# Haochen-Wang409/U2PL

Hardware: AMD Instinct MI355X
Metric: train images/sec at 769x769 (R101-DeepLabv3+) (higher is better)
Workload: dtype f32

## Files before the change

### u2pl_amd/csrc/nn.hip

```cpp
#include "common.h"
#include "u2pl_hip.h"

__device__ __forceinline__ float4 f4add(float4 a, float4 b) { return make_float4(a.x + b.x, a.y + b.y, a.z + b.z, a.w + b.w); }
__device__ __forceinline__ float4 f4mul(float4 a, float4 b) { return make_float4(a.x * b.x, a.y * b.y, a.z * b.z, a.w * b.w); }
__device__ __forceinline__ float4 f4sub(float4 a, float4 b) { return make_float4(a.x - b.x, a.y - b.y, a.z - b.z, a.w - b.w); }
__device__ __forceinline__ float4 f4zero() { return make_float4(0.f, 0.f, 0.f, 0.f); }

struct StatOp {
    const float* x; long ld; const float* pivot;
    __device__ __forceinline__ void get(long row, int c4, float4& v0, float4& v1) const {
        float4 v = *(const float4*)(x + row * ld + c4 * 4);
        if (pivot) v = f4sub(v, *(const float4*)(pivot + c4 * 4));
        v0 = v; v1 = f4mul(v, v);
    }
};
struct SumOp {
    const float* x; long ld;
    __device__ __forceinline__ void get(long row, int c4, float4& v0, float4& v1) const {
        v0 = *(const float4*)(x + row * ld + c4 * 4); v1 = f4zero();
    }
};
__device__ __forceinline__ float4 relu_mask_from_x(float4 g, float4 xv, const float* mean, const float* invstd, const float* gamma,
                                                   const float* beta, int c) {
    const float4 mu = *(const float4*)(mean + c), is = *(const float4*)(invstd + c), ga = *(const float4*)(gamma + c), be = *(const float4*)(beta + c);
    g.x = ((xv.x - mu.x) * is.x * ga.x + be.x) > 0.f ? g.x : 0.f;
    g.y = ((xv.y - mu.y) * is.y * ga.y + be.y) > 0.f ? g.y : 0.f;
    g.z = ((xv.z - mu.z) * is.z * ga.z + be.z) > 0.f ? g.z : 0.f;
    g.w = ((xv.w - mu.w) * is.w * ga.w + be.w) > 0.f ? g.w : 0.f;
    return g;
}
struct BnBwdOp {
    const float* dy; long lddy; const float* x; long ldx; const float* y; long ldy;
    const float* mean; const float* invstd; const float* drop; long rows_per_image; int C;
    const float* gamma; const float* relu_beta;
    __device__ __forceinline__ void get(long row, int c4, float4& v0, float4& v1) const {
        float4 g = *(const float4*)(dy + row * lddy + c4 * 4);
        float4 xv = *(const float4*)(x + row * ldx + c4 * 4);
        if (y) {
            float4 yy = *(const float4*)(y + row * ldy + c4 * 4);
            g.x = yy.x > 0.f ? g.x : 0.f; g.y = yy.y > 0.f ? g.y : 0.f;
            g.z = yy.z > 0.f ? g.z : 0.f; g.w = yy.w > 0.f ? g.w : 0.f;
        } else if (relu_beta) {
            g = relu_mask_from_x(g, xv, mean, invstd, gamma, relu_beta, c4 * 4);
        }
        if (drop) g = f4mul(g, *(const float4*)(drop + (row / rows_per_image) * C + c4 * 4));
        float4 xh = f4mul(f4sub(xv, *(const float4*)(mean + c4 * 4)), *(const float4*)(invstd + c4 * 4));
        v0 = g; v1 = f4mul(g, xh);
    }
};

template <class Op>
__global__ U2PL_HBM_KERNEL void k_colreduce_partial(Op op, long Mseg, int C, float* __restrict__ partial) {
    __shared__ float4 sh0[256], sh1[256];
    const int C4 = C >> 2;
    const int slab0 = blockIdx.z * 64;
    const int wcols = min(64, C4 - slab0);
    const int tc = wcols, tr = 256 / tc;
    const int tid = threadIdx.x, cl = tid % tc, rg = tid / tc;
    const int nblk = gridDim.x, seg = blockIdx.y;
    const long per = (Mseg + nblk - 1) / nblk;
    const long rb = seg * Mseg + blockIdx.x * per, re = min(seg * Mseg + Mseg, rb + per);
    float* out = partial + ((long)seg * nblk + blockIdx.x) * 2 * C;
    const int c4 = slab0 + cl;
    float4 a0 = f4zero(), a1 = f4zero();
    if (rg < tr) {
        float4 b0 = f4zero(), b1 = f4zero(), c0 = f4zero(), c1 = f4zero(), d0 = f4zero(), d1 = f4zero();
        long r = rb + rg;
        for (; r + 3 * (long)tr < re; r += 4 * (long)tr) {
            float4 v0, v1, w0, w1, x0, x1, y0, y1;
            op.get(r, c4, v0, v1);
            op.get(r + tr, c4, w0, w1);
            op.get(r + 2 * (long)tr, c4, x0, x1);
            op.get(r + 3 * (long)tr, c4, y0, y1);
            a0 = f4add(a0, v0); a1 = f4add(a1, v1);
            b0 = f4add(b0, w0); b1 = f4add(b1, w1);
            c0 = f4add(c0, x0); c1 = f4add(c1, x1);
            d0 = f4add(d0, y0); d1 = f4add(d1, y1);
        }
        for (; r < re; r += tr) {
            float4 v0, v1;
            op.get(r, c4, v0, v1);
            a0 = f4add(a0, v0); a1 = f4add(a1, v1);
        }
        a0 = f4add(f4add(a0, b0), f4add(c0, d0));
        a1 = f4add(f4add(a1, b1), f4add(c1, d1));
    }
    sh0[tid] = a0; sh1[tid] = a1;
    __syncthreads();
    if (rg == 0) {
        for (int k = 1; k < tr; ++k) { a0 = f4add(a0, sh0[k * tc + cl]); a1 = f4add(a1, sh1[k * tc + cl]); }
        *(float4*)(out + c4 * 4) = a0;
        *(float4*)(out + C + c4 * 4) = a1;
    }
}
__global__ __launch_bounds__(1024) void k_colreduce_final(const float* __restrict__ partial, int nblk, int C,
                                                          double* __restrict__ out) {
    __shared__ double sh[16][64];
    const int seg = blockIdx.y;
    const int cl = threadIdx.x & 63, rg = threadIdx.x >> 6;
    const int i = blockIdx.x * 64 + cl;
    double acc = 0.0;
    if (i < 2 * C) {
        const float* p = partial + (long)seg * nblk * 2 * C + i;
        int b = rg;
        for (; b + 7 * 16 < nblk; b += 8 * 16) {
            float v[8];
#pragma unroll
            for (int u = 0; u < 8; ++u) v[u] = p[(long)(b + u * 16) * 2 * C];
#pragma unroll
            for (int u = 0; u < 8; ++u) acc += (double)v[u];
        }
        for (; b < nblk; b += 16) acc += (double)p[(long)b * 2 * C];
    }
    sh[rg][cl] = acc;
    __syncthreads();
    if (rg == 0 && i < 2 * C) {
        double t = 0.0;
#pragma unroll
        for (int k = 0; k < 16; ++k) t += sh[k][cl];
        out[(long)seg * 2 * C + i] = t;
    }
}
static int colreduce_blocks(long Mseg) {
    long b = (Mseg + 63) / 64;
    return (int)(b < 1 ? 1 : (b > 512 ? 512 : b));
}
U2PL_API size_t u2pl_colreduce_workspace_bytes(long Mseg, int nseg, int C) {
    return (size_t)nseg * colreduce_blocks(Mseg) * 2 * C * sizeof(float);
}
template <class Op>
static int run_colreduce(Op op, long Mseg, int nseg, int C, void* ws, double* out, hipStream_t stream) {
    if (C % 4 || Mseg <= 0) return U2PL_EINVAL;
    const int nblk = colreduce_blocks(Mseg);
    U2PL_LAUNCH((k_colreduce_partial<Op>), dim3(nblk, nseg, cdiv(C / 4, 64)), dim3(256), 0, stream, op, Mseg, C, (float*)ws);
    U2PL_LAUNCH_CHECK();
    U2PL_LAUNCH(k_colreduce_final, dim3(cdiv(2 * C, 64), nseg), dim3(1024), 0, stream, (const float*)ws, nblk, C, out);
    U2PL_LAUNCH_CHECK();
    return 0;
}

U2PL_API int u2pl_colreduce_finish_f32(const float* partial, int nblk, int C, double* sums, hipStream_t stream) {
    U2PL_LAUNCH(k_colreduce_final, dim3(cdiv(2 * C, 64), 1), dim3(1024), 0, stream, partial, nblk, C, sums);
    U2PL_LAUNCH_CHECK();
    return 0;
}

__global__ void k_bn_stats_small(const float* __restrict__ x, long ld, int M, int C, const float* __restrict__ pivot,
                                 double* __restrict__ sums) {
    const int c = blockIdx.x * blockDim.x + threadIdx.x;
    if (c >= C) return;
    double s = 0.0;
    for (int m = 0; m < M; ++m) s += (double)x[m * ld + c];
    const double mean = s / M;
    double q = 0.0;
    for (int m = 0; m < M; ++m) { const double d = (double)x[m * ld + c] - mean; q += d * d; }
    const double dm = mean - (pivot ? (double)pivot[c] : 0.0);
    sums[c] = M * dm;
    sums[C + c] = q + M * dm * dm;
}
U2PL_API int u2pl_bn_stats_f32(const float* x, long ld, long M, int C, const float* pivot, void* workspace,
                               double* sums, hipStream_t stream) {
    if (M <= 64) {
        U2PL_LAUNCH(k_bn_stats_small, dim3(cdiv(C, 64)), dim3(64), 0, stream, x, ld, (int)M, C, pivot, sums);
        U2PL_LAUNCH_CHECK();
        return 0;
    }
    StatOp op = {x, ld, pivot};
    return run_colreduce(op, M, 1, C, workspace, sums, stream);
}
U2PL_API int u2pl_colsum_f32(const float* x, long ld, long Mseg, int nseg, int C, void* workspace, double* sums,
                             hipStream_t stream) {
    SumOp op = {x, ld};
    return run_colreduce(op, Mseg, nseg, C, workspace, sums, stream);
}
U2PL_API int u2pl_bn_bwd_sums_f32(const float* dy, long lddy, const float* x, long ldx, const float* y, long ldy,
                                  const float* mean, const float* invstd, const float* drop, long rows_per_image,
                                  long M, int C, void* workspace, double* sums, hipStream_t stream) {
    BnBwdOp op = {dy, lddy, x, ldx, y, ldy, mean, invstd, drop, rows_per_image, C, nullptr, nullptr};
    return run_colreduce(op, M, 1, C, workspace, sums, stream);
}
U2PL_API int u2pl_bn_bwd_sums_mx_f32(const float* dy, long lddy, const float* x, long ldx, const float* mean, const float* invstd,
                                     const float* gamma, const float* beta, const float* drop, long rows_per_image, long M, int C,
                                     void* workspace, double* sums, hipStream_t stream) {
    if (!gamma || !beta) return U2PL_EINVAL;
    BnBwdOp op = {dy, lddy, x, ldx, nullptr, 0, mean, invstd, drop, rows_per_image, C, gamma, beta};
    return run_colreduce(op, M, 1, C, workspace, sums, stream);
}

__global__ void k_bn_finalize(const double* __restrict__ sums, double count, const float* __restrict__ pivot, int C,
                              float eps, float momentum, float* __restrict__ mean, float* __restrict__ invstd,
                              float* __restrict__ running_mean, float* __restrict__ running_var) {
    for (int c = blockIdx.x * blockDim.x + threadIdx.x; c < C; c += gridDim.x * blockDim.x) {
        const double m1 = sums[c] / count, m2 = sums[C + c] / count;
        const double p = pivot ? (double)pivot[c] : 0.0;
        double var = m2 - m1 * m1;
        if (var < 0.0) var = 0.0;
        const double mu = p + m1;
        mean[c] = (float)mu;
        invstd[c] = (float)(1.0 / sqrt(var + (double)eps));
        if (running_mean) {
            const double unb = count > 1.0 ? var * count / (count - 1.0) : var;
            running_mean[c] = (float)((1.0 - momentum) * running_mean[c] + momentum * mu);
            running_var[c] = (float)((1.0 - momentum) * running_var[c] + momentum * unb);
        }
    }
}
U2PL_API int u2pl_bn_finalize_f32(const double* sums, double count, const float* pivot, int C, float eps,
                                  float momentum, float* mean, float* invstd, float* running_mean,
                                  float* running_var, hipStream_t stream) {
    U2PL_LAUNCH(k_bn_finalize, dim3(cdiv(C, 256)), dim3(256), 0, stream, sums, count, pivot, C, eps, momentum,
                       mean, invstd, running_mean, running_var);
    U2PL_LAUNCH_CHECK();
    return 0;
}
__global__ __launch_bounds__(1024) void k_bn_finish_finalize(const float* __restrict__ partial, int nblk, int C, double count,
                                                             const float* __restrict__ pivot, float eps, float momentum,
                                                             float* __restrict__ mean, float* __restrict__ invstd,
                                                             float* __restrict__ running_mean, float* __restrict__ running_var,
                                                             double* __restrict__ sums_out) {
    __shared__ double sh[16][64];
    __shared__ double tot[64];
    const int cl = threadIdx.x & 63, rg = threadIdx.x >> 6;
    const int c = blockIdx.x * 32 + (cl & 31);
    const int i = (cl >> 5) * C + c;
    double acc = 0.0;
    if (c < C) {
        const float* p = partial + i;
        int b = rg;
        for (; b + 7 * 16 < nblk; b += 8 * 16) {
            float v[8];
#pragma unroll
            for (int u = 0; u < 8; ++u) v[u] = p[(long)(b + u * 16) * 2 * C];
#pragma unroll
            for (int u = 0; u < 8; ++u) acc += (double)v[u];
        }
        for (; b < nblk; b += 16) acc += (double)p[(long)b * 2 * C];
    }
    sh[rg][cl] = acc;
    __syncthreads();
    if (rg == 0) {
        double t = 0.0;
#pragma unroll
        for (int k = 0; k < 16; ++k) t += sh[k][cl];
        tot[cl] = t;
        if (sums_out && c < C) sums_out[i] = t;
    }
    __syncthreads();
    if (threadIdx.x < 32 && c < C) {
        const double m1 = tot[cl] / count, m2 = tot[32 + cl] / count;
        const double pv = pivot ? (double)pivot[c] : 0.0;
        double var = m2 - m1 * m1;
        if (var < 0.0) var = 0.0;
        const double mu = pv + m1;
        mean[c] = (float)mu;
        invstd[c] = (float)(1.0 / sqrt(var + (double)eps));
        if (running_mean) {
            const double unb = count > 1.0 ? var * count / (count - 1.0) : var;
            running_mean[c] = (float)((1.0 - momentum) * running_mean[c] + momentum * mu);
            running_var[c] = (float)((1.0 - momentum) * running_var[c] + momentum * unb);
        }
    }
}
U2PL_API int u2pl_bn_finish_finalize_f32(const float* partial, int nblk, int C, double count, const float* pivot, float eps,
                                         float momentum, float* mean, float* invstd, float* running_mean, float* running_var,
                                         double* sums_out, hipStream_t stream) {
    if (!partial || nblk <= 0 || C <= 0 || !mean || !invstd) return U2PL_EINVAL;
    U2PL_LAUNCH(k_bn_finish_finalize, dim3(cdiv(C, 32)), dim3(1024), 0, stream, partial, nblk, C, count, pivot, eps, momentum, mean,
                invstd, running_mean, running_var, sums_out);
    U2PL_LAUNCH_CHECK();
    return 0;
}
__global__ void k_bn_eval_prep(const float* __restrict__ rv, int C, float eps, float* __restrict__ invstd) {
    for (int c = blockIdx.x * blockDim.x + threadIdx.x; c < C; c += gridDim.x * blockDim.x)
        invstd[c] = (float)(1.0 / sqrt((double)rv[c] + (double)eps));
}
U2PL_API int u2pl_bn_eval_invstd_f32(const float* running_var, int C, float eps, float* invstd, hipStream_t stream) {
    U2PL_LAUNCH(k_bn_eval_prep, dim3(cdiv(C, 256)), dim3(256), 0, stream, running_var, C, eps, invstd);
    U2PL_LAUNCH_CHECK();
    return 0;
}

struct EvalPrepJob { const float* rv; float* out; long long begin; int C; float eps; };
__global__ void k_bn_eval_prep_multi(const EvalPrepJob* __restrict__ jobs, int njobs, long total) {
    for (long e = blockIdx.x * (long)blockDim.x + threadIdx.x; e < total; e += (long)gridDim.x * blockDim.x) {
        int lo = 0, hi = njobs - 1;
        while (lo < hi) {
            const int mid = (lo + hi + 1) >> 1;
            if (jobs[mid].begin <= e) lo = mid; else hi = mid - 1;
        }
        const EvalPrepJob j = jobs[lo];
        const int c = (int)(e - j.begin);
        if (c < j.C) j.out[c] = (float)(1.0 / sqrt((double)j.rv[c] + (double)j.eps));
    }
}
U2PL_API size_t u2pl_bn_eval_invstd_job_bytes(void) { return sizeof(EvalPrepJob); }
U2PL_API int u2pl_bn_eval_invstd_multi_f32(const void* jobs_dev, int njobs, long total, hipStream_t stream) {
    if (njobs <= 0 || total <= 0) return 0;
    if (!jobs_dev) return U2PL_EINVAL;
    U2PL_LAUNCH(k_bn_eval_prep_multi, dim3(grid_for(total, 256)), dim3(256), 0, stream, (const EvalPrepJob*)jobs_dev, njobs, total);
    U2PL_LAUNCH_CHECK();
    return 0;
}

__global__ U2PL_HBM_KERNEL void k_bn_apply(const float* __restrict__ x, long ldx, const float* __restrict__ mean,
                           const float* __restrict__ invstd, const float* __restrict__ gamma,
                           const float* __restrict__ beta, const float* __restrict__ res, long ldr, int relu,
                           const float* __restrict__ drop, long rows_per_image, float* __restrict__ y, long ldy,
                           long M, int C, unsigned* __restrict__ y_amax) {
    const int C4 = C >> 2;
    const long total = M * C4;
    unsigned am = 0u;
    for (long i = blockIdx.x * (long)blockDim.x + threadIdx.x; i < total; i += (long)gridDim.x * blockDim.x) {
        const long r = i / C4;
        const int c = (int)(i % C4) * 4;
        float4 v = *(const float4*)(x + r * ldx + c);
        const float4 mu = *(const float4*)(mean + c), is = *(const float4*)(invstd + c);
        const float4 ga = *(const float4*)(gamma + c), be = *(const float4*)(beta + c);
        v.x = (v.x - mu.x) * is.x * ga.x + be.x; v.y = (v.y - mu.y) * is.y * ga.y + be.y;
        v.z = (v.z - mu.z) * is.z * ga.z + be.z; v.w = (v.w - mu.w) * is.w * ga.w + be.w;
        if (res) v = f4add(v, *(const float4*)(res + r * ldr + c));
        if (relu) { v.x = fmaxf(v.x, 0.f); v.y = fmaxf(v.y, 0.f); v.z = fmaxf(v.z, 0.f); v.w = fmaxf(v.w, 0.f); }
        if (drop) v = f4mul(v, *(const float4*)(drop + (r / rows_per_image) * C + c));
        *(float4*)(y + r * ldy + c) = v;
        am = amax_bits4(am, v);
    }
    if (y_amax) amax_wave_publish(am, y_amax);
}
U2PL_API int u2pl_bn_apply_f32(const float* x, long ldx, const float* mean, const float* invstd, const float* gamma,
                               const float* beta, const float* res, long ldr, int relu, const float* drop,
                               long rows_per_image, float* y, long ldy, long M, int C, hipStream_t stream) {
    if (C % 4) return U2PL_EINVAL;
    U2PL_LAUNCH(k_bn_apply, dim3(grid_for(M * (C / 4), 256)), dim3(256), 0, stream, x, ldx, mean, invstd, gamma,
                       beta, res, ldr, relu, drop, rows_per_image, y, ldy, M, C, (unsigned*)nullptr);
    U2PL_LAUNCH_CHECK();
    return 0;
}
U2PL_API int u2pl_bn_apply_amax_f32(const float* x, long ldx, const float* mean, const float* invstd, const float* gamma,
                                    const float* beta, const float* res, long ldr, int relu, const float* drop,
                                    long rows_per_image, float* y, long ldy, long M, int C, float* y_amax, hipStream_t stream) {
    if (C % 4) return U2PL_EINVAL;
    U2PL_LAUNCH(k_bn_apply, dim3(grid_for(M * (C / 4), 256)), dim3(256), 0, stream, x, ldx, mean, invstd, gamma,
                       beta, res, ldr, relu, drop, rows_per_image, y, ldy, M, C, (unsigned*)y_amax);
    U2PL_LAUNCH_CHECK();
    return 0;
}

__global__ U2PL_HBM_KERNEL void k_bn_bwd_apply(const float* __restrict__ dy, long lddy, const float* __restrict__ x, long ldx,
                               const float* __restrict__ y, long ldy, const float* __restrict__ mean,
                               const float* __restrict__ invstd, const float* __restrict__ gamma,
                               const float* __restrict__ drop, long rows_per_image,
                               const double* __restrict__ sums, double count, float* __restrict__ dx, long lddx,
                               float* __restrict__ dres, long lddr, long M, int C, const double* __restrict__ psums,
                               float* __restrict__ gsink, float* __restrict__ bsink, int accumulate,
                               unsigned* __restrict__ dx_amax, unsigned* __restrict__ dres_amax, const float* __restrict__ relu_beta) {
    unsigned am_x = 0u, am_r = 0u;
    if (psums) {
        for (long i = blockIdx.x * (long)blockDim.x + threadIdx.x; i < C; i += (long)gridDim.x * blockDim.x) {
            gsink[i] = (accumulate ? gsink[i] : 0.f) + (float)(psums[C + i] * (double)1.0f);
            bsink[i] = (accumulate ? bsink[i] : 0.f) + (float)(psums[i] * (double)1.0f);
        }
    }
    const int C4 = C >> 2;
    const long total = M * C4;
    for (long i = blockIdx.x * (long)blockDim.x + threadIdx.x; i < total; i += (long)gridDim.x * blockDim.x) {
        const long r = i / C4;
        const int c = (int)(i % C4) * 4;
        float4 g = *(const float4*)(dy + r * lddy + c);
        if (y) {
            const float4 yy = *(const float4*)(y + r * ldy + c);
            g.x = yy.x > 0.f ? g.x : 0.f; g.y = yy.y > 0.f ? g.y : 0.f;
            g.z = yy.z > 0.f ? g.z : 0.f; g.w = yy.w > 0.f ? g.w : 0.f;
        } else if (relu_beta) {
            g = relu_mask_from_x(g, *(const float4*)(x + r * ldx + c), mean, invstd, gamma, relu_beta, c);
        }
        if (drop) g = f4mul(g, *(const float4*)(drop + (r / rows_per_image) * C + c));
        if (dres) *(float4*)(dres + r * lddr + c) = g;
        am_r = amax_bits4(am_r, g);
        const float4 is = *(const float4*)(invstd + c), ga = *(const float4*)(gamma + c);
        float4 o;
        if (sums) {
            const float4 xv = *(const float4*)(x + r * ldx + c), mu = *(const float4*)(mean + c);
            const float m0x = (float)(sums[c] / count), m0y = (float)(sums[c + 1] / count);
            const float m0z = (float)(sums[c + 2] / count), m0w = (float)(sums[c + 3] / count);
            const float m1x = (float)(sums[C + c] / count), m1y = (float)(sums[C + c + 1] / count);
            const float m1z = (float)(sums[C + c + 2] / count), m1w = (float)(sums[C + c + 3] / count);
            o.x = ga.x * is.x * (g.x - m0x - (xv.x - mu.x) * is.x * m1x);
            o.y = ga.y * is.y * (g.y - m0y - (xv.y - mu.y) * is.y * m1y);
            o.z = ga.z * is.z * (g.z - m0z - (xv.z - mu.z) * is.z * m1z);
            o.w = ga.w * is.w * (g.w - m0w - (xv.w - mu.w) * is.w * m1w);
        } else {
            o = f4mul(f4mul(ga, is), g);
        }
        *(float4*)(dx + r * lddx + c) = o;
        am_x = amax_bits4(am_x, o);
    }
    if (dx_amax) amax_wave_publish(am_x, dx_amax);
    if (dres_amax) amax_wave_publish(am_r, dres_amax);
}
U2PL_API int u2pl_bn_bwd_apply_f32(const float* dy, long lddy, const float* x, long ldx, const float* y, long ldy,
                                   const float* mean, const float* invstd, const float* gamma, const float* drop,
                                   long rows_per_image, const double* sums, double count, float* dx, long lddx,
                                   float* dres, long lddr, long M, int C, hipStream_t stream) {
    if (C % 4) return U2PL_EINVAL;
    U2PL_LAUNCH(k_bn_bwd_apply, dim3(grid_for(M * (C / 4), 256)), dim3(256), 0, stream, dy, lddy, x, ldx, y, ldy,
                       mean, invstd, gamma, drop, rows_per_image, sums, count, dx, lddx, dres, lddr, M, C, (const double*)nullptr,
                       (float*)nullptr, (float*)nullptr, 0, (unsigned*)nullptr, (unsigned*)nullptr, (const float*)nullptr);
    U2PL_LAUNCH_CHECK();
    return 0;
}
U2PL_API int u2pl_bn_bwd_apply_pg_f32(const float* dy, long lddy, const float* x, long ldx, const float* y, long ldy,
                                      const float* mean, const float* invstd, const float* gamma, const float* drop,
                                      long rows_per_image, const double* sums, double count, float* dx, long lddx,
                                      float* dres, long lddr, long M, int C, const double* psums, float* gsink, float* bsink,
                                      int accumulate, hipStream_t stream) {
    if (C % 4 || !psums || !gsink || !bsink) return U2PL_EINVAL;
    U2PL_LAUNCH(k_bn_bwd_apply, dim3(grid_for(M * (C / 4), 256)), dim3(256), 0, stream, dy, lddy, x, ldx, y, ldy,
                       mean, invstd, gamma, drop, rows_per_image, sums, count, dx, lddx, dres, lddr, M, C, psums, gsink, bsink,
                       accumulate, (unsigned*)nullptr, (unsigned*)nullptr, (const float*)nullptr);
    U2PL_LAUNCH_CHECK();
    return 0;
}
U2PL_API int u2pl_bn_bwd_apply_amax_f32(const float* dy, long lddy, const float* x, long ldx, const float* y, long ldy,
                                        const float* mean, const float* invstd, const float* gamma, const float* drop,
                                        long rows_per_image, const double* sums, double count, float* dx, long lddx,
                                        float* dres, long lddr, long M, int C, const double* psums, float* gsink, float* bsink,
                                        int accumulate, float* dx_amax, float* dres_amax, const float* relu_beta, hipStream_t stream) {
    if (C % 4 || (psums && (!gsink || !bsink)) || (relu_beta && y)) return U2PL_EINVAL;
    U2PL_LAUNCH(k_bn_bwd_apply, dim3(grid_for(M * (C / 4), 256)), dim3(256), 0, stream, dy, lddy, x, ldx, y, ldy,
                       mean, invstd, gamma, drop, rows_per_image, sums, count, dx, lddx, dres, lddr, M, C, psums, gsink, bsink,
                       accumulate, (unsigned*)dx_amax, (unsigned*)dres_amax, relu_beta);
    U2PL_LAUNCH_CHECK();
    return 0;
}
__global__ void k_sums_to_f32(const double* __restrict__ s, int n, float scale, int accumulate, float* __restrict__ out) {
    for (int i = blockIdx.x * blockDim.x + threadIdx.x; i < n; i += gridDim.x * blockDim.x)
        out[i] = (accumulate ? out[i] : 0.f) + (float)(s[i] * (double)scale);
}
U2PL_API int u2pl_sums_to_f32(const double* sums, int n, float scale, int accumulate, float* out, hipStream_t stream) {
    U2PL_LAUNCH(k_sums_to_f32, dim3(cdiv(n, 256)), dim3(256), 0, stream, sums, n, scale, accumulate, out);
    U2PL_LAUNCH_CHECK();
    return 0;
}

__global__ void k_maxpool_fwd(const float* __restrict__ x, long ldx, int N, int H, int W, int C, int Ho, int Wo,
                              float* __restrict__ y, long ldy, unsigned char* __restrict__ tap) {
    const int C4 = C >> 2;
    const long total = (long)N * Ho * Wo * C4;
    for (long i = blockIdx.x * (long)blockDim.x + threadIdx.x; i < total; i += (long)gridDim.x * blockDim.x) {
        const int c = (int)(i % C4) * 4;
        long p = i / C4;
        const int wo = (int)(p % Wo);
        long t = p / Wo;
        const int ho = (int)(t % Ho), n = (int)(t / Ho);
        float4 best = make_float4(-INFINITY, -INFINITY, -INFINITY, -INFINITY);
        uchar4 bt = make_uchar4(0, 0, 0, 0);
        bool first = true;
        for (int r = 0; r < 3; ++r) {
            const int ih = ho * 2 - 1 + r;
            if (ih < 0 || ih >= H) continue;
            for (int s = 0; s < 3; ++s) {
                const int iw = wo * 2 - 1 + s;
                if (iw < 0 || iw >= W) continue;
                const float4 v = *(const float4*)(x + ((long)(n * H + ih) * W + iw) * ldx + c);
                const unsigned char k = (unsigned char)(r * 3 + s);
                if (first || v.x > best.x || v.x != v.x) { best.x = v.x; bt.x = k; }
                if (first || v.y > best.y || v.y != v.y) { best.y = v.y; bt.y = k; }
                if (first || v.z > best.z || v.z != v.z) { best.z = v.z; bt.z = k; }
                if (first || v.w > best.w || v.w != v.w) { best.w = v.w; bt.w = k; }
                first = false;
            }
        }
        *(float4*)(y + p * ldy + c) = best;
        *(uchar4*)(tap + p * C + c) = bt;
    }
}
U2PL_API int u2pl_maxpool3s2_fwd_f32(const float* x, long ldx, int N, int H, int W, int C, int Ho, int Wo, float* y,
                                     long ldy, unsigned char* tap, hipStream_t stream) {
    if (C % 4) return U2PL_EINVAL;
    U2PL_LAUNCH(k_maxpool_fwd, dim3(grid_for((long)N * Ho * Wo * (C / 4), 256)), dim3(256), 0, stream, x, ldx, N, H,
                       W, C, Ho, Wo, y, ldy, tap);
    U2PL_LAUNCH_CHECK();
    return 0;
}
__global__ void k_maxpool_bwd(const float* __restrict__ dy, long lddy, const unsigned char* __restrict__ tap, int N,
                              int H, int W, int C, int Ho, int Wo, float* __restrict__ dx, long lddx) {
    const int C4 = C >> 2;
    const long total = (long)N * H * W * C4;
    for (long i = blockIdx.x * (long)blockDim.x + threadIdx.x; i < total; i += (long)gridDim.x * blockDim.x) {
        const int c = (int)(i % C4) * 4;
        long p = i / C4;
        const int iw = (int)(p % W);
        long t = p / W;
        const int ih = (int)(t % H), n = (int)(t / H);
        float4 acc = f4zero();
        for (int ho = ih / 2; ho <= (ih + 1) / 2; ++ho) {
            if (ho >= Ho) continue;
            const int r = ih - (ho * 2 - 1);
            if (r < 0 || r > 2) continue;
            for (int wo = iw / 2; wo <= (iw + 1) / 2; ++wo) {
                if (wo >= Wo) continue;
                const int s = iw - (wo * 2 - 1);
                if (s < 0 || s > 2) continue;
                const long q = ((long)n * Ho + ho) * Wo + wo;
                const uchar4 k = *(const uchar4*)(tap + q * C + c);
                const float4 g = *(const float4*)(dy + q * lddy + c);
                const unsigned char me = (unsigned char)(r * 3 + s);
                if (k.x == me) acc.x += g.x;
                if (k.y == me) acc.y += g.y;
                if (k.z == me) acc.z += g.z;
                if (k.w == me) acc.w += g.w;
            }
        }
        *(float4*)(dx + p * lddx + c) = acc;
    }
}
U2PL_API int u2pl_maxpool3s2_bwd_f32(const float* dy, long lddy, const unsigned char* tap, int N, int H, int W, int C,
                                     int Ho, int Wo, float* dx, long lddx, hipStream_t stream) {
    U2PL_LAUNCH(k_maxpool_bwd, dim3(grid_for((long)N * H * W * (C / 4), 256)), dim3(256), 0, stream, dy, lddy, tap, N,
                       H, W, C, Ho, Wo, dx, lddx);
    U2PL_LAUNCH_CHECK();
    return 0;
}

__global__ void k_copy_rows(const float* __restrict__ src, long lds, float* __restrict__ dst, long ldd, long M, int C,
                            int accumulate) {
    const int C4 = C >> 2;
    const long total = M * C4;
    for (long i = blockIdx.x * (long)blockDim.x + threadIdx.x; i < total; i += (long)gridDim.x * blockDim.x) {
        const long r = i / C4;
        const int c = (int)(i % C4) * 4;
        float4 v = *(const float4*)(src + r * lds + c);
        if (accumulate) v = f4add(v, *(const float4*)(dst + r * ldd + c));
        *(float4*)(dst + r * ldd + c) = v;
    }
}
U2PL_API int u2pl_copy_rows_f32(const float* src, long lds, float* dst, long ldd, long M, int C, int accumulate,
                                hipStream_t stream) {
    if (C % 4) return U2PL_EINVAL;
    if (M <= 0) return 0;
    U2PL_LAUNCH(k_copy_rows, dim3(grid_for(M * (C / 4), 256)), dim3(256), 0, stream, src, lds, dst, ldd, M, C, accumulate);
    U2PL_LAUNCH_CHECK();
    return 0;
}
__global__ void k_copy_cols(const float* __restrict__ src, long lds, float* __restrict__ dst, long ldd, long M, int C) {
    const long total = M * C;
    for (long i = blockIdx.x * (long)blockDim.x + threadIdx.x; i < total; i += (long)gridDim.x * blockDim.x) {
        const long r = i / C;
        const int c = (int)(i % C);
        dst[r * ldd + c] = src[r * lds + c];
    }
}
U2PL_API int u2pl_copy_cols_f32(const float* src, long lds, float* dst, long ldd, long M, int C, hipStream_t stream) {
    if (M <= 0) return 0;
    U2PL_LAUNCH(k_copy_cols, dim3(grid_for(M * C, 256)), dim3(256), 0, stream, src, lds, dst, ldd, M, C);
    U2PL_LAUNCH_CHECK();
    return 0;
}
__global__ void k_broadcast_rows(const float* __restrict__ v, long ldv, float scale, float* __restrict__ dst, long ldd,
                                 long rows_per_image, long M, int C) {
    const int C4 = C >> 2;
    const long total = M * C4;
    for (long i = blockIdx.x * (long)blockDim.x + threadIdx.x; i < total; i += (long)gridDim.x * blockDim.x) {
        const long r = i / C4;
        const int c = (int)(i % C4) * 4;
        float4 a = *(const float4*)(v + (r / rows_per_image) * ldv + c);
        a.x *= scale; a.y *= scale; a.z *= scale; a.w *= scale;
        *(float4*)(dst + r * ldd + c) = a;
    }
}
U2PL_API int u2pl_broadcast_rows_f32(const float* v, long ldv, float scale, float* dst, long ldd, long rows_per_image,
                                     long M, int C, hipStream_t stream) {
    if (C % 4) return U2PL_EINVAL;
    U2PL_LAUNCH(k_broadcast_rows, dim3(grid_for(M * (C / 4), 256)), dim3(256), 0, stream, v, ldv, scale, dst, ldd,
                       rows_per_image, M, C);
    U2PL_LAUNCH_CHECK();
    return 0;
}

__global__ void k_bilinear_rows_fwd(const float* __restrict__ x, long ldx, int N, int h, int w, int C, int H, int W,
                                    float sy, float sx, float* __restrict__ y, long ldy) {
    const int C4 = C >> 2;
    const long total = (long)N * H * W * C4;
    for (long i = blockIdx.x * (long)blockDim.x + threadIdx.x; i < total; i += (long)gridDim.x * blockDim.x) {
        const int c = (int)(i % C4) * 4;
        long p = i / C4;
        const int ox = (int)(p % W);
        long t = p / W;
        const int oy = (int)(t % H), n = (int)(t / H);
        const AcCoord cy = ac_coord(oy, sy, h), cx = ac_coord(ox, sx, w);
        const float* b = x + (long)n * h * w * ldx + c;
        const float4 v00 = *(const float4*)(b + ((long)cy.i0 * w + cx.i0) * ldx), v01 = *(const float4*)(b + ((long)cy.i0 * w + cx.i1) * ldx);
        const float4 v10 = *(const float4*)(b + ((long)cy.i1 * w + cx.i0) * ldx), v11 = *(const float4*)(b + ((long)cy.i1 * w + cx.i1) * ldx);
        float4 o;
#define BL(f) o.f = __fmaf_rn(cy.l0, __fmaf_rn(cx.l0, v00.f, __fmul_rn(cx.l1, v01.f)), __fmul_rn(cy.l1, __fmaf_rn(cx.l0, v10.f, __fmul_rn(cx.l1, v11.f))))
        BL(x); BL(y); BL(z); BL(w);
#undef BL
        *(float4*)(y + p * ldy + c) = o;
    }
}
U2PL_API int u2pl_bilinear_rows_fwd_f32(const float* x, long ldx, int N, int h, int w, int C, int H, int W, float* y,
                                        long ldy, hipStream_t stream) {
    if (C % 4) return U2PL_EINVAL;
    U2PL_LAUNCH(k_bilinear_rows_fwd, dim3(grid_for((long)N * H * W * (C / 4), 256)), dim3(256), 0, stream, x, ldx, N, h,
                       w, C, H, W, ac_scale_host(h, H), ac_scale_host(w, W), y, ldy);
    U2PL_LAUNCH_CHECK();
    return 0;
}
__global__ void k_bilinear_rows_bwd(const float* __restrict__ dy, long lddy, int N, int h, int w, int C, int H, int W,
                                    float sy, float sx, float* __restrict__ dx, long lddx) {
    const int C4 = C >> 2;
    const long total = (long)N * h * w * C4;
    for (long i = blockIdx.x * (long)blockDim.x + threadIdx.x; i < total; i += (long)gridDim.x * blockDim.x) {
        const int c = (int)(i % C4) * 4;
        long p = i / C4;
        const int ix = (int)(p % w);
        long t = p / w;
        const int iy = (int)(t % h), n = (int)(t / h);
        int oy_lo = sy > 0 ? (int)floorf((iy - 1) / sy) - 1 : 0, oy_hi = sy > 0 ? (int)ceilf((iy + 1) / sy) + 1 : H - 1;
        int ox_lo = sx > 0 ? (int)floorf((ix - 1) / sx) - 1 : 0, ox_hi = sx > 0 ? (int)ceilf((ix + 1) / sx) + 1 : W - 1;
        oy_lo = max(oy_lo, 0); ox_lo = max(ox_lo, 0);
        oy_hi = min(oy_hi, H - 1); ox_hi = min(ox_hi, W - 1);
        float4 acc = f4zero();
        for (int oy = oy_lo; oy <= oy_hi; ++oy) {
            const AcCoord cy = ac_coord(oy, sy, h);
            if (cy.i0 != iy && cy.i1 != iy) continue;
            const float wy = (cy.i0 == iy ? cy.l0 : 0.f) + (cy.i1 == iy ? cy.l1 : 0.f);
            for (int ox = ox_lo; ox <= ox_hi; ++ox) {
                const AcCoord cx = ac_coord(ox, sx, w);
                if (cx.i0 != ix && cx.i1 != ix) continue;
                const float ww = wy * ((cx.i0 == ix ? cx.l0 : 0.f) + (cx.i1 == ix ? cx.l1 : 0.f));
                const float4 g = *(const float4*)(dy + (((long)n * H + oy) * W + ox) * lddy + c);
                acc.x += ww * g.x; acc.y += ww * g.y; acc.z += ww * g.z; acc.w += ww * g.w;
            }
        }
        *(float4*)(dx + p * lddx + c) = acc;
    }
}
U2PL_API int u2pl_bilinear_rows_bwd_f32(const float* dy, long lddy, int N, int h, int w, int C, int H, int W, float* dx,
                                        long lddx, hipStream_t stream) {
    if (C % 4) return U2PL_EINVAL;
    U2PL_LAUNCH(k_bilinear_rows_bwd, dim3(grid_for((long)N * h * w * (C / 4), 256)), dim3(256), 0, stream, dy, lddy, N,
                       h, w, C, H, W, ac_scale_host(h, H), ac_scale_host(w, W), dx, lddx);
    U2PL_LAUNCH_CHECK();
    return 0;
}

__global__ void k_softmax_rows(const float* __restrict__ x, long ldx, float* __restrict__ y, long ldy, long M, int C) {
    for (long r = blockIdx.x * (long)blockDim.x + threadIdx.x; r < M; r += (long)gridDim.x * blockDim.x) {
        const float* b = x + r * ldx;
        float m = b[0];
        for (int c = 1; c < C; ++c) m = fmaxf(m, b[c]);
        float s = 0.f;
        for (int c = 0; c < C; ++c) s += expf(b[c] - m);
        for (int c = 0; c < C; ++c) y[r * ldy + c] = expf(b[c] - m) / s;
    }
}
U2PL_API int u2pl_softmax_rows_f32(const float* x, long ldx, float* y, long ldy, long M, int C, hipStream_t stream) {
    U2PL_LAUNCH(k_softmax_rows, dim3(grid_for(M, 256)), dim3(256), 0, stream, x, ldx, y, ldy, M, C);
    U2PL_LAUNCH_CHECK();
    return 0;
}

__global__ void k_sgd(float* __restrict__ p, const float* __restrict__ g, float* __restrict__ buf, long n, long b1,
                      long b2, float lr0, float lr1, float lr2, float mom, float wd, int first, float gscale) {
    for (long i = blockIdx.x * (long)blockDim.x + threadIdx.x; i < n; i += (long)gridDim.x * blockDim.x) {
        const float lr = i < b1 ? lr0 : (i < b2 ? lr1 : lr2);
        const float pv = p[i];
        const float gv = __fadd_rn(__fmul_rn(g[i], gscale), __fmul_rn(wd, pv));
        const float bv = first ? gv : __fadd_rn(__fmul_rn(mom, buf[i]), gv);
        buf[i] = bv;
        p[i] = __fsub_rn(pv, __fmul_rn(lr, bv));
    }
}
U2PL_API int u2pl_sgd_step_f32(float* p, const float* g, float* buf, long n, long b1, long b2, float lr0, float lr1,
                               float lr2, float momentum, float weight_decay, int first, float grad_scale,
                               hipStream_t stream) {
    if (n <= 0) return 0;
    U2PL_LAUNCH(k_sgd, dim3(grid_for(n, 256)), dim3(256), 0, stream, p, g, buf, n, b1, b2, lr0, lr1, lr2, momentum,
                       weight_decay, first, grad_scale);
    U2PL_LAUNCH_CHECK();
    return 0;
}
__global__ void k_adam(float* __restrict__ p, const float* __restrict__ g, float* __restrict__ m, float* __restrict__ v, long n,
                       long b1, long b2, float lr0, float lr1, float lr2, float beta1, float beta2, float eps, float wd,
                       float bc1, float bc2s, float gscale) {
    for (long i = blockIdx.x * (long)blockDim.x + threadIdx.x; i < n; i += (long)gridDim.x * blockDim.x) {
        const float lr = i < b1 ? lr0 : (i < b2 ? lr1 : lr2);
        const float pv = p[i];
        const float gv = __fadd_rn(__fmul_rn(g[i], gscale), __fmul_rn(wd, pv));
        const float mv = __fadd_rn(m[i], __fmul_rn(1.0f - beta1, __fsub_rn(gv, m[i])));
        const float vv = __fadd_rn(__fmul_rn(v[i], beta2), __fmul_rn(1.0f - beta2, __fmul_rn(gv, gv)));
        m[i] = mv;
        v[i] = vv;
        const float denom = __fadd_rn(__fdiv_rn(__fsqrt_rn(vv), bc2s), eps);
        p[i] = __fsub_rn(pv, __fmul_rn(__fdiv_rn(lr, bc1), __fdiv_rn(mv, denom)));
    }
}
U2PL_API int u2pl_adam_step_f32(float* p, const float* g, float* exp_avg, float* exp_avg_sq, long n, long b1, long b2,
                                float lr0, float lr1, float lr2, float beta1, float beta2, float eps, float weight_decay,
                                float bias_correction1, float bias_correction2_sqrt, float grad_scale, hipStream_t stream) {
    if (n <= 0) return 0;
    if (!(bias_correction1 > 0.f) || !(bias_correction2_sqrt > 0.f)) return U2PL_EINVAL;
    U2PL_LAUNCH(k_adam, dim3(grid_for(n, 256)), dim3(256), 0, stream, p, g, exp_avg, exp_avg_sq, n, b1, b2, lr0, lr1, lr2, beta1,
                beta2, eps, weight_decay, bias_correction1, bias_correction2_sqrt, grad_scale);
    U2PL_LAUNCH_CHECK();
    return 0;
}
__global__ void k_ema(float* __restrict__ t, const float* __restrict__ s, long n, float d, float omd) {
    for (long i = blockIdx.x * (long)blockDim.x + threadIdx.x; i < n; i += (long)gridDim.x * blockDim.x)
        t[i] = __fadd_rn(__fmul_rn(d, t[i]), __fmul_rn(omd, s[i]));
}
U2PL_API int u2pl_ema_update_f32(float* t, const float* s, long n, float decay, float one_minus_decay,
                                 hipStream_t stream) {
    if (n <= 0) return 0;
    U2PL_LAUNCH(k_ema, dim3(grid_for(n, 256)), dim3(256), 0, stream, t, s, n, decay, one_minus_decay);
    U2PL_LAUNCH_CHECK();
    return 0;
}

#define DENSE_MAXM 16
__global__ __launch_bounds__(256) void k_dense_small(const float* __restrict__ x, long ldx, const float* __restrict__ w,
                                                     const float* __restrict__ bias, float* __restrict__ y, long ldy,
                                                     int M, int K, int Cout) {
    const int o = blockIdx.x * 4 + (threadIdx.x >> 6), lane = threadIdx.x & 63;
    if (o >= Cout) return;
    double acc[DENSE_MAXM];
#pragma unroll
    for (int m = 0; m < DENSE_MAXM; ++m) acc[m] = 0.0;
    const float* wr = w + (long)o * K;
    for (int k = lane * 4; k < K; k += 256) {
        const float4 wv = *(const float4*)(wr + k);
#pragma unroll
// ... 204 lines not shown
```

Before: 35.95.

## Restructure BN apply kernels into channel-slab row walks with unrolled loads

The forward and backward BN apply kernels drop the flat grid-stride loop, which needed a division and modulo per element and reloaded per-channel parameters every iteration. Each block now owns a slab of up to 64 float4 channel columns and a range of rows. Per-channel constants (mean, invstd, gamma, beta, and the backward sums/count divisions) are loaded once per thread, and four rows are loaded together to raise memory-level parallelism. The grid is capped at 4096 blocks. For narrow channel counts some threads sit idle, and register pressure rises with the unroll.

```diff
diff --git a/u2pl_amd/csrc/nn.hip b/u2pl_amd/csrc/nn.hip
--- a/u2pl_amd/csrc/nn.hip
+++ b/u2pl_amd/csrc/nn.hip
@@ -302,55 +302,135 @@
     return 0;
 }
 
-__global__ U2PL_HBM_KERNEL void k_bn_apply(const float* __restrict__ x, long ldx, const float* __restrict__ mean,
+#ifndef U2PL_BN_ROWS
+#define U2PL_BN_ROWS 4
+#endif
+struct BnWalk { int c; int tr; long r0, re; bool on; };
+__device__ __forceinline__ BnWalk bn_walk(long M, int C4, int nslab) {
+    const int slab = (int)(blockIdx.x % (unsigned)nslab), rblk = (int)(blockIdx.x / (unsigned)nslab);
+    const int nrb = (int)(gridDim.x / (unsigned)nslab);
+    const int slab0 = slab * 64;
+    const int tc = min(64, C4 - slab0), tr = 256 / tc;
+    const int cl = (int)threadIdx.x % tc, rg = (int)threadIdx.x / tc;
+    const long per = (M + nrb - 1) / nrb;
+    const long rb = rblk * per;
+    BnWalk w;
+    w.c = (slab0 + cl) * 4; w.tr = tr; w.r0 = rb + rg; w.re = min(M, rb + per); w.on = rg < tr;
+    return w;
+}
+static int bn_walk_grid(long M, int C, int* nslab_out) {
+    const int C4 = C / 4, nslab = cdiv(C4, 64);
+    const int tr = 256 / (C4 < 64 ? C4 : 64);
+    long nrb = (M + (long)tr * U2PL_BN_ROWS - 1) / ((long)tr * U2PL_BN_ROWS);
+    const long cap = 4096 / nslab > 1 ? 4096 / nslab : 1;
+    if (nrb > cap) nrb = cap;
+    if (nrb < 1) nrb = 1;
+    *nslab_out = nslab;
+    return (int)nrb * nslab;
+}
+
+__device__ __forceinline__ float4 bn_apply_one(float4 v, float4 mu, float4 is, float4 ga, float4 be, bool has_res, float4 rs,
+                                               int relu, const float* __restrict__ drop, long r, long rows_per_image, int C, int c) {
+    v.x = (v.x - mu.x) * is.x * ga.x + be.x; v.y = (v.y - mu.y) * is.y * ga.y + be.y;
+    v.z = (v.z - mu.z) * is.z * ga.z + be.z; v.w = (v.w - mu.w) * is.w * ga.w + be.w;
+    if (has_res) v = f4add(v, rs);
+    if (relu) { v.x = fmaxf(v.x, 0.f); v.y = fmaxf(v.y, 0.f); v.z = fmaxf(v.z, 0.f); v.w = fmaxf(v.w, 0.f); }
+    if (drop) v = f4mul(v, *(const float4*)(drop + (r / rows_per_image) * C + c));
+    return v;
+}
+__global__ U2PL_HBM_KERNEL __launch_bounds__(256) void k_bn_apply(const float* __restrict__ x, long ldx, const float* __restrict__ mean,
                            const float* __restrict__ invstd, const float* __restrict__ gamma,
                            const float* __restrict__ beta, const float* __restrict__ res, long ldr, int relu,
                            const float* __restrict__ drop, long rows_per_image, float* __restrict__ y, long ldy,
-                           long M, int C, unsigned* __restrict__ y_amax) {
-    const int C4 = C >> 2;
-    const long total = M * C4;
+                           long M, int C, int nslab, unsigned* __restrict__ y_amax) {
     unsigned am = 0u;
-    for (long i = blockIdx.x * (long)blockDim.x + threadIdx.x; i < total; i += (long)gridDim.x * blockDim.x) {
-        const long r = i / C4;
-        const int c = (int)(i % C4) * 4;
-        float4 v = *(const float4*)(x + r * ldx + c);
+    const BnWalk w = bn_walk(M, C >> 2, nslab);
+    if (w.on) {
+        const int c = w.c;
+        const long tr = w.tr;
         const float4 mu = *(const float4*)(mean + c), is = *(const float4*)(invstd + c);
         const float4 ga = *(const float4*)(gamma + c), be = *(const float4*)(beta + c);
-        v.x = (v.x - mu.x) * is.x * ga.x + be.x; v.y = (v.y - mu.y) * is.y * ga.y + be.y;
-        v.z = (v.z - mu.z) * is.z * ga.z + be.z; v.w = (v.w - mu.w) * is.w * ga.w + be.w;
-        if (res) v = f4add(v, *(const float4*)(res + r * ldr + c));
-        if (relu) { v.x = fmaxf(v.x, 0.f); v.y = fmaxf(v.y, 0.f); v.z = fmaxf(v.z, 0.f); v.w = fmaxf(v.w, 0.f); }
-        if (drop) v = f4mul(v, *(const float4*)(drop + (r / rows_per_image) * C + c));
-        *(float4*)(y + r * ldy + c) = v;
-        am = amax_bits4(am, v);
+        const bool has_res = res != nullptr;
+        long r = w.r0;
+        for (; r + (U2PL_BN_ROWS - 1) * tr < w.re; r += U2PL_BN_ROWS * tr) {
+            float4 v[U2PL_BN_ROWS], rs[U2PL_BN_ROWS];
+#pragma unroll
+            for (int u = 0; u < U2PL_BN_ROWS; ++u) v[u] = *(const float4*)(x + (r + u * tr) * ldx + c);
+#pragma unroll
+            for (int u = 0; u < U2PL_BN_ROWS; ++u) rs[u] = has_res ? *(const float4*)(res + (r + u * tr) * ldr + c) : f4zero();
+#pragma unroll
+            for (int u = 0; u < U2PL_BN_ROWS; ++u) {
+                v[u] = bn_apply_one(v[u], mu, is, ga, be, has_res, rs[u], relu, drop, r + u * tr, rows_per_image, C, c);
+                *(float4*)(y + (r + u * tr) * ldy + c) = v[u];
+                am = amax_bits4(am, v[u]);
+            }
+        }
+        for (; r < w.re; r += tr) {
+            float4 v = *(const float4*)(x + r * ldx + c);
+            const float4 rs = has_res ? *(const float4*)(res + r * ldr + c) : f4zero();
+            v = bn_apply_one(v, mu, is, ga, be, has_res, rs, relu, drop, r, rows_per_image, C, c);
+            *(float4*)(y + r * ldy + c) = v;
+            am = amax_bits4(am, v);
+        }
     }
     if (y_amax) amax_wave_publish(am, y_amax);
 }
 U2PL_API int u2pl_bn_apply_f32(const float* x, long ldx, const float* mean, const float* invstd, const float* gamma,
                                const float* beta, const float* res, long ldr, int relu, const float* drop,
                                long rows_per_image, float* y, long ldy, long M, int C, hipStream_t stream) {
-    if (C % 4) return U2PL_EINVAL;
-    U2PL_LAUNCH(k_bn_apply, dim3(grid_for(M * (C / 4), 256)), dim3(256), 0, stream, x, ldx, mean, invstd, gamma,
-                       beta, res, ldr, relu, drop, rows_per_image, y, ldy, M, C, (unsigned*)nullptr);
+    if (C % 4 || C <= 0) return U2PL_EINVAL;
+    int nslab;
+    const int grid = bn_walk_grid(M, C, &nslab);
+    U2PL_LAUNCH(k_bn_apply, dim3(grid), dim3(256), 0, stream, x, ldx, mean, invstd, gamma,
+                       beta, res, ldr, relu, drop, rows_per_image, y, ldy, M, C, nslab, (unsigned*)nullptr);
     U2PL_LAUNCH_CHECK();
     return 0;
 }
 U2PL_API int u2pl_bn_apply_amax_f32(const float* x, long ldx, const float* mean, const float* invstd, const float* gamma,
                                     const float* beta, const float* res, long ldr, int relu, const float* drop,
                                     long rows_per_image, float* y, long ldy, long M, int C, float* y_amax, hipStream_t stream) {
-    if (C % 4) return U2PL_EINVAL;
-    U2PL_LAUNCH(k_bn_apply, dim3(grid_for(M * (C / 4), 256)), dim3(256), 0, stream, x, ldx, mean, invstd, gamma,
-                       beta, res, ldr, relu, drop, rows_per_image, y, ldy, M, C, (unsigned*)y_amax);
-    U2PL_LAUNCH_CHECK();
-    return 0;
-}
-
-__global__ U2PL_HBM_KERNEL void k_bn_bwd_apply(const float* __restrict__ dy, long lddy, const float* __restrict__ x, long ldx,
+    if (C % 4 || C <= 0) return U2PL_EINVAL;
+    int nslab;
+    const int grid = bn_walk_grid(M, C, &nslab);
+    U2PL_LAUNCH(k_bn_apply, dim3(grid), dim3(256), 0, stream, x, ldx, mean, invstd, gamma,
+                       beta, res, ldr, relu, drop, rows_per_image, y, ldy, M, C, nslab, (unsigned*)y_amax);
+    U2PL_LAUNCH_CHECK();
+    return 0;
+}
+
+struct BnBwdCh { float4 mu, is, ga, rb, m0, m1; };
+__device__ __forceinline__ float4 bn_bwd_g(float4 g, bool ymask, float4 yy, bool xmask, float4 xv, const BnBwdCh& k,
+                                           const float* __restrict__ drop, long r, long rows_per_image, int C, int c) {
+    if (ymask) {
+        g.x = yy.x > 0.f ? g.x : 0.f; g.y = yy.y > 0.f ? g.y : 0.f;
+        g.z = yy.z > 0.f ? g.z : 0.f; g.w = yy.w > 0.f ? g.w : 0.f;
+    } else if (xmask) {
+        g.x = ((xv.x - k.mu.x) * k.is.x * k.ga.x + k.rb.x) > 0.f ? g.x : 0.f;
+        g.y = ((xv.y - k.mu.y) * k.is.y * k.ga.y + k.rb.y) > 0.f ? g.y : 0.f;
+        g.z = ((xv.z - k.mu.z) * k.is.z * k.ga.z + k.rb.z) > 0.f ? g.z : 0.f;
+        g.w = ((xv.w - k.mu.w) * k.is.w * k.ga.w + k.rb.w) > 0.f ? g.w : 0.f;
+    }
+    if (drop) g = f4mul(g, *(const float4*)(drop + (r / rows_per_image) * C + c));
+    return g;
+}
+__device__ __forceinline__ float4 bn_bwd_dx(float4 g, bool train, float4 xv, const BnBwdCh& k) {
+    float4 o;
+    if (train) {
+        o.x = k.ga.x * k.is.x * (g.x - k.m0.x - (xv.x - k.mu.x) * k.is.x * k.m1.x);
+        o.y = k.ga.y * k.is.y * (g.y - k.m0.y - (xv.y - k.mu.y) * k.is.y * k.m1.y);
+        o.z = k.ga.z * k.is.z * (g.z - k.m0.z - (xv.z - k.mu.z) * k.is.z * k.m1.z);
+        o.w = k.ga.w * k.is.w * (g.w - k.m0.w - (xv.w - k.mu.w) * k.is.w * k.m1.w);
+    } else {
+        o = f4mul(f4mul(k.ga, k.is), g);
+    }
+    return o;
+}
+__global__ U2PL_HBM_KERNEL __launch_bounds__(256) void k_bn_bwd_apply(const float* __restrict__ dy, long lddy, const float* __restrict__ x, long ldx,
                                const float* __restrict__ y, long ldy, const float* __restrict__ mean,
                                const float* __restrict__ invstd, const float* __restrict__ gamma,
                                const float* __restrict__ drop, long rows_per_image,
                                const double* __restrict__ sums, double count, float* __restrict__ dx, long lddx,
-                               float* __restrict__ dres, long lddr, long M, int C, const double* __restrict__ psums,
+                               float* __restrict__ dres, long lddr, long M, int C, int nslab, const double* __restrict__ psums,
                                float* __restrict__ gsink, float* __restrict__ bsink, int accumulate,
                                unsigned* __restrict__ dx_amax, unsigned* __restrict__ dres_amax, const float* __restrict__ relu_beta) {
     unsigned am_x = 0u, am_r = 0u;
@@ -360,39 +440,54 @@
             bsink[i] = (accumulate ? bsink[i] : 0.f) + (float)(psums[i] * (double)1.0f);
         }
     }
-    const int C4 = C >> 2;
-    const long total = M * C4;
-    for (long i = blockIdx.x * (long)blockDim.x + threadIdx.x; i < total; i += (long)gridDim.x * blockDim.x) {
-        const long r = i / C4;
-        const int c = (int)(i % C4) * 4;
-        float4 g = *(const float4*)(dy + r * lddy + c);
-        if (y) {
-            const float4 yy = *(const float4*)(y + r * ldy + c);
-            g.x = yy.x > 0.f ? g.x : 0.f; g.y = yy.y > 0.f ? g.y : 0.f;
-            g.z = yy.z > 0.f ? g.z : 0.f; g.w = yy.w > 0.f ? g.w : 0.f;
-        } else if (relu_beta) {
-            g = relu_mask_from_x(g, *(const float4*)(x + r * ldx + c), mean, invstd, gamma, relu_beta, c);
-        }
-        if (drop) g = f4mul(g, *(const float4*)(drop + (r / rows_per_image) * C + c));
-        if (dres) *(float4*)(dres + r * lddr + c) = g;
-        am_r = amax_bits4(am_r, g);
-        const float4 is = *(const float4*)(invstd + c), ga = *(const float4*)(gamma + c);
-        float4 o;
-        if (sums) {
-            const float4 xv = *(const float4*)(x + r * ldx + c), mu = *(const float4*)(mean + c);
-            const float m0x = (float)(sums[c] / count), m0y = (float)(sums[c + 1] / count);
-            const float m0z = (float)(sums[c + 2] / count), m0w = (float)(sums[c + 3] / count);
-            const float m1x = (float)(sums[C + c] / count), m1y = (float)(sums[C + c + 1] / count);
-            const float m1z = (float)(sums[C + c + 2] / count), m1w = (float)(sums[C + c + 3] / count);
-            o.x = ga.x * is.x * (g.x - m0x - (xv.x - mu.x) * is.x * m1x);
-            o.y = ga.y * is.y * (g.y - m0y - (xv.y - mu.y) * is.y * m1y);
-            o.z = ga.z * is.z * (g.z - m0z - (xv.z - mu.z) * is.z * m1z);
-            o.w = ga.w * is.w * (g.w - m0w - (xv.w - mu.w) * is.w * m1w);
-        } else {
-            o = f4mul(f4mul(ga, is), g);
-        }
-        *(float4*)(dx + r * lddx + c) = o;
-        am_x = amax_bits4(am_x, o);
+    const BnWalk w = bn_walk(M, C >> 2, nslab);
+    if (w.on) {
+        const int c = w.c;
+        const long tr = w.tr;
+        const bool ymask = y != nullptr, xmask = !ymask && relu_beta != nullptr, train = sums != nullptr;
+        const bool need_x = xmask || train;
+        BnBwdCh k;
+        k.is = *(const float4*)(invstd + c); k.ga = *(const float4*)(gamma + c);
+        k.mu = need_x ? *(const float4*)(mean + c) : f4zero();
+        k.rb = xmask ? *(const float4*)(relu_beta + c) : f4zero();
+        k.m0 = f4zero(); k.m1 = f4zero();
+        if (train) {
+            k.m0.x = (float)(sums[c] / count); k.m0.y = (float)(sums[c + 1] / count);
+            k.m0.z = (float)(sums[c + 2] / count); k.m0.w = (float)(sums[c + 3] / count);
+            k.m1.x = (float)(sums[C + c] / count); k.m1.y = (float)(sums[C + c + 1] / count);
+            k.m1.z = (float)(sums[C + c + 2] / count); k.m1.w = (float)(sums[C + c + 3] / count);
+        }
+        long r = w.r0;
+        for (; r + (U2PL_BN_ROWS - 1) * tr < w.re; r += U2PL_BN_ROWS * tr) {
+            float4 g[U2PL_BN_ROWS], yy[U2PL_BN_ROWS], xv[U2PL_BN_ROWS];
+#pragma unroll
+            for (int u = 0; u < U2PL_BN_ROWS; ++u) g[u] = *(const float4*)(dy + (r + u * tr) * lddy + c);
+#pragma unroll
+            for (int u = 0; u < U2PL_BN_ROWS; ++u) yy[u] = ymask ? *(const float4*)(y + (r + u * tr) * ldy + c) : f4zero();
+#pragma unroll
+            for (int u = 0; u < U2PL_BN_ROWS; ++u) xv[u] = need_x ? *(const float4*)(x + (r + u * tr) * ldx + c) : f4zero();
+#pragma unroll
+            for (int u = 0; u < U2PL_BN_ROWS; ++u) {
+                const long ru = r + u * tr;
+                g[u] = bn_bwd_g(g[u], ymask, yy[u], xmask, xv[u], k, drop, ru, rows_per_image, C, c);
+                if (dres) *(float4*)(dres + ru * lddr + c) = g[u];
+                am_r = amax_bits4(am_r, g[u]);
+                const float4 o = bn_bwd_dx(g[u], train, xv[u], k);
+                *(float4*)(dx + ru * lddx + c) = o;
+                am_x = amax_bits4(am_x, o);
+            }
+        }
+        for (; r < w.re; r += tr) {
+            float4 g = *(const float4*)(dy + r * lddy + c);
+            const float4 yy = ymask ? *(const float4*)(y + r * ldy + c) : f4zero();
+            const float4 xv = need_x ? *(const float4*)(x + r * ldx + c) : f4zero();
+            g = bn_bwd_g(g, ymask, yy, xmask, xv, k, drop, r, rows_per_image, C, c);
+            if (dres) *(float4*)(dres + r * lddr + c) = g;
+            am_r = amax_bits4(am_r, g);
+            const float4 o = bn_bwd_dx(g, train, xv, k);
+            *(float4*)(dx + r * lddx + c) = o;
+            am_x = amax_bits4(am_x, o);
+        }
     }
     if (dx_amax) amax_wave_publish(am_x, dx_amax);
     if (dres_amax) amax_wave_publish(am_r, dres_amax);
@@ -401,9 +496,10 @@
                                    const float* mean, const float* invstd, const float* gamma, const float* drop,
                                    long rows_per_image, const double* sums, double count, float* dx, long lddx,
                                    float* dres, long lddr, long M, int C, hipStream_t stream) {
-    if (C % 4) return U2PL_EINVAL;
-    U2PL_LAUNCH(k_bn_bwd_apply, dim3(grid_for(M * (C / 4), 256)), dim3(256), 0, stream, dy, lddy, x, ldx, y, ldy,
-                       mean, invstd, gamma, drop, rows_per_image, sums, count, dx, lddx, dres, lddr, M, C, (const double*)nullptr,
+    if (C % 4 || C <= 0) return U2PL_EINVAL;
+    int nslab;
+    U2PL_LAUNCH(k_bn_bwd_apply, dim3(bn_walk_grid(M, C, &nslab)), dim3(256), 0, stream, dy, lddy, x, ldx, y, ldy,
+                       mean, invstd, gamma, drop, rows_per_image, sums, count, dx, lddx, dres, lddr, M, C, nslab, (const double*)nullptr,
                        (float*)nullptr, (float*)nullptr, 0, (unsigned*)nullptr, (unsigned*)nullptr, (const float*)nullptr);
     U2PL_LAUNCH_CHECK();
     return 0;
@@ -413,9 +509,10 @@
                                       long rows_per_image, const double* sums, double count, float* dx, long lddx,
                                       float* dres, long lddr, long M, int C, const double* psums, float* gsink, float* bsink,
                                       int accumulate, hipStream_t stream) {
-    if (C % 4 || !psums || !gsink || !bsink) return U2PL_EINVAL;
-    U2PL_LAUNCH(k_bn_bwd_apply, dim3(grid_for(M * (C / 4), 256)), dim3(256), 0, stream, dy, lddy, x, ldx, y, ldy,
-                       mean, invstd, gamma, drop, rows_per_image, sums, count, dx, lddx, dres, lddr, M, C, psums, gsink, bsink,
+    if (C % 4 || C <= 0 || !psums || !gsink || !bsink) return U2PL_EINVAL;
+    int nslab;
+    U2PL_LAUNCH(k_bn_bwd_apply, dim3(bn_walk_grid(M, C, &nslab)), dim3(256), 0, stream, dy, lddy, x, ldx, y, ldy,
+                       mean, invstd, gamma, drop, rows_per_image, sums, count, dx, lddx, dres, lddr, M, C, nslab, psums, gsink, bsink,
                        accumulate, (unsigned*)nullptr, (unsigned*)nullptr, (const float*)nullptr);
     U2PL_LAUNCH_CHECK();
     return 0;
@@ -425,9 +522,10 @@
                                         long rows_per_image, const double* sums, double count, float* dx, long lddx,
                                         float* dres, long lddr, long M, int C, const double* psums, float* gsink, float* bsink,
                                         int accumulate, float* dx_amax, float* dres_amax, const float* relu_beta, hipStream_t stream) {
-    if (C % 4 || (psums && (!gsink || !bsink)) || (relu_beta && y)) return U2PL_EINVAL;
-    U2PL_LAUNCH(k_bn_bwd_apply, dim3(grid_for(M * (C / 4), 256)), dim3(256), 0, stream, dy, lddy, x, ldx, y, ldy,
-                       mean, invstd, gamma, drop, rows_per_image, sums, count, dx, lddx, dres, lddr, M, C, psums, gsink, bsink,
+    if (C % 4 || C <= 0 || (psums && (!gsink || !bsink)) || (relu_beta && y)) return U2PL_EINVAL;
+    int nslab;
+    U2PL_LAUNCH(k_bn_bwd_apply, dim3(bn_walk_grid(M, C, &nslab)), dim3(256), 0, stream, dy, lddy, x, ldx, y, ldy,
+                       mean, invstd, gamma, drop, rows_per_image, sums, count, dx, lddx, dres, lddr, M, C, nslab, psums, gsink, bsink,
                        accumulate, (unsigned*)dx_amax, (unsigned*)dres_amax, relu_beta);
     U2PL_LAUNCH_CHECK();
     return 0;
```

New measurement: 36.74 (median of 6 runs). 1.02x the previous value.
